# linum-uqam/ViT-OCM-WMSegmentation

Measured on NVIDIA B200. Metric: sliding_window_seg_megapixels_per_s, higher is better.
Workload: dtype fp16

## Files before the change

### vit-ocm-wmsegmentation_b200/csrc/attention_quad_sm100.cuh

```cuda
#pragma once
#include "attention_sm100.cuh"

namespace vitocm {

constexpr int AQ_PIPES = 4;
constexpr int AQ_BKV = 64;
constexpr int AQ_RING = 5;
constexpr int AQ_TILE_BYTES = AQ_BKV * ATT_DH * 2;
constexpr int AQ_Q_BYTES = ATT_BQ * ATT_DH * 2;
constexpr int AQ_THREADS = (4 * AQ_PIPES + 4) * 32;
constexpr int AQ_PIPE_SMEM = AQ_Q_BYTES + AQ_RING * AQ_TILE_BYTES;
constexpr int AQ_PIPE_BARS = 128;
constexpr int AQ_SMEM_BYTES = AQ_PIPES * (AQ_PIPE_SMEM + AQ_PIPE_BARS) + 64 + 1024 ;
constexpr int AQ_REGS_SOFTMAX = 104;
constexpr int AQ_REGS_CTRL = 64;
static_assert(16 * AQ_REGS_SOFTMAX + 4 * AQ_REGS_CTRL <= 20 * 96, "quad attention: setmaxnreg budgets exceed the launch allocation");
static_assert(AQ_SMEM_BYTES <= 227 * 1024, "quad attention: shared memory");
constexpr int AQ_S_COL = 0;
constexpr int AQ_O_COL = 64;

__device__ __forceinline__ void aq_decode(const AttnArgs& a, int it, int& pair0, int& qt, int& nslots) {
  if (a.group_items == 0) {
    pair0 = it / a.n_fullq;
    qt = it - pair0 * a.n_fullq;
    nslots = 1;
    return;
  }
  const int g = it / a.group_items, r = it - g * a.group_items;
  if (r < a.pack * a.n_fullq) {
    const int pi = r / a.n_fullq;
    pair0 = g * a.pack + pi;
    qt = r - pi * a.n_fullq;
    nslots = 1;
  } else {
    pair0 = g * a.pack;
    qt = a.n_fullq;
    nslots = a.pack;
  }
}
template <int NS, int SL>
__device__ __forceinline__ void aq_slot_mask(uint32_t (&m)[4]) {
#pragma unroll
  for (int w = 0; w < 4; ++w) m[w] = ((NS == 4 ? w : (NS == 2 ? (w >> 1) : 0)) == SL) ? 0u : 0xffffffffu;
}

template <bool F16, bool TL = false>
__global__ void __launch_bounds__(AQ_THREADS, 1)
attn_fwd_quad_kernel(const __grid_constant__ CUtensorMap tmap_q , const __grid_constant__ CUtensorMap tmap_kv ,
                     const __grid_constant__ CUtensorMap tmap_q32 , const AttnArgs args) {
  extern __shared__ __align__(1024) uint8_t smem_raw[];
  const uint32_t smem = (ptx::smem_u32(smem_raw) + 1023u) & ~1023u;
  const uint32_t bars0 = smem + AQ_PIPES * AQ_PIPE_SMEM;
  const uint32_t tmem_ptr_smem = bars0 + AQ_PIPES * AQ_PIPE_BARS;
  const int warp = threadIdx.x >> 5;
  const int lane = threadIdx.x & 31;
  const int N = args.n_tokens;
  const int D = args.embed_dim;
  const int n_kv = (N + AQ_BKV - 1) / AQ_BKV;
  const int p = warp < 4 * AQ_PIPES ? (warp >> 2) : (warp - 4 * AQ_PIPES);
  const uint32_t smem_q = smem + p * AQ_PIPE_SMEM;
  const uint32_t smem_ring = smem_q + AQ_Q_BYTES;
  const uint32_t bars = bars0 + p * AQ_PIPE_BARS;
  const uint32_t q_full = bars;
  const uint32_t s_full = bars + 8;
  const uint32_t p_full = bars + 16;
  const uint32_t o_full = bars + 24;
  const uint32_t o_empty = bars + 32;
  const uint32_t kv_full = bars + 40;
  const uint32_t kv_empty = bars + 80;
  static_assert(80 + 8 * AQ_RING <= AQ_PIPE_BARS, "quad attention: barrier block");

  if (warp == 4 * AQ_PIPES && lane == 0) {
    ptx::prefetch_tmap(&tmap_q);
    ptx::prefetch_tmap(&tmap_kv);
    ptx::prefetch_tmap(&tmap_q32);
    for (int pp = 0; pp < AQ_PIPES; ++pp) {
      const uint32_t b = bars0 + pp * AQ_PIPE_BARS;
      ptx::mbar_init(b, 1);
      ptx::mbar_init(b + 8, 1);
      ptx::mbar_init(b + 16, 4);
      ptx::mbar_init(b + 24, 1);
      ptx::mbar_init(b + 32, 4);
      for (int i = 0; i < AQ_RING; ++i) {
        ptx::mbar_init(b + 40 + 8 * i, 1);
        ptx::mbar_init(b + 80 + 8 * i, 1);
      }
    }
    ptx::fence_barrier_init();
  }
  if (warp == 4 * AQ_PIPES + 1) {
    ptx::tmem_alloc(tmem_ptr_smem, 512);
    ptx::tmem_relinquish();
  }
  if (warp == 4 * AQ_PIPES + 2 && lane == 0 && args.stagger_clk > 0) {
    const long long wait_clk = static_cast<long long>(args.stagger_clk) * blockIdx.x / gridDim.x;
    const long long t0 = clock64();
    while (clock64() - t0 < wait_clk) {}
  }
  ptx::tc_fence_before();
  __syncthreads();
  ptx::tc_fence_after();
  const uint32_t tmem_base = ptx::lds_u32(tmem_ptr_smem) + static_cast<uint32_t>(p * 128);

  const int first = static_cast<int>(blockIdx.x) * AQ_PIPES + p;
  const int stride = static_cast<int>(gridDim.x) * AQ_PIPES;

  if (warp >= 4 * AQ_PIPES) {
    asm volatile("setmaxnreg.dec.sync.aligned.u32 %0;" ::"n"(AQ_REGS_CTRL));
    if (ptx::elect_one()) {
      const uint32_t s_tmem = tmem_base + AQ_S_COL, o_tmem = tmem_base + AQ_O_COL;
      const uint64_t q_desc = ptx::make_smem_desc_sw128(smem_q, 1024, 0);
      auto kv_len_mma = [&](int j) {
        int len = N - j * AQ_BKV;
        len = len > AQ_BKV ? AQ_BKV : len;
        return (len + 15) & ~15;
      };
      auto clamp_pair = [&](int pr) { return pr < args.n_pairs ? pr : args.n_pairs - 1; };
      auto load_q = [&](int it) {
        int pair0, qt, ns;
        aq_decode(args, it, pair0, qt, ns);
        ptx::mbar_arrive_expect_tx(q_full, AQ_Q_BYTES);
        if (ns == 1) {
          const int pair = clamp_pair(pair0);
          const int b = pair / args.heads, h = pair - b * args.heads;
          ptx::tma_load_2d(smem_q, &tmap_q, q_full, h * ATT_DH, b * N + qt * ATT_BQ);
        } else {
          const int per = 4 / ns;
          for (int u = 0; u < 4; ++u) {
            const int pr = clamp_pair(pair0 + u / per);
            const int b = pr / args.heads, h = pr - b * args.heads;
            ptx::tma_load_2d(smem_q + u * 4096, &tmap_q32, q_full, h * ATT_DH, b * N + qt * ATT_BQ + (u % per) * 32);
          }
        }
      };
      int loaded = 0, used = 0;
      int l_it = first, l_j = 0, l_which = 1, l_sl = 0, l_ns = 1;
      int l_col = 0, l_row = 0;
      auto set_load_coords = [&]() {
        if (l_it < args.n_items) {
          int pair0, qt;
          aq_decode(args, l_it, pair0, qt, l_ns);
          const int pr = clamp_pair(pair0 + l_sl);
          const int b = pr / args.heads;
          l_col = (pr - b * args.heads) * ATT_DH;
          l_row = b * N;
        }
      };
      set_load_coords();
      auto fill = [&]() {
        while (loaded - used < AQ_RING && l_it < args.n_items) {
          const int slot = loaded % AQ_RING;
          if (loaded >= AQ_RING) ptx::mbar_wait(kv_empty + 8 * slot, ((loaded / AQ_RING) - 1) & 1, 50);
          ptx::mbar_arrive_expect_tx(kv_full + 8 * slot, AQ_TILE_BYTES);
          ptx::tma_load_2d(smem_ring + slot * AQ_TILE_BYTES, &tmap_kv, kv_full + 8 * slot, l_which * D + l_col, l_row + l_j * AQ_BKV);
          ++loaded;
          bool recode = l_ns > 1;
          if (++l_sl == l_ns) {
            l_sl = 0;
            if (l_which == 1) {
              l_which = 2;
            } else {
              l_which = 1;
              if (++l_j == n_kv) { l_j = 0; l_it += stride; recode = true; }
            }
          }
          if (recode) set_load_coords();
        }
      };
      if (first < args.n_items) load_q(first);
      fill();
      auto issue_s = [&](int j, int nslots) {
        const uint32_t idesc = ptx::make_idesc(ATT_BQ, kv_len_mma(j), false, false, F16 ? 0u : 1u);
        if (nslots == 1) {
          const int slot = used % AQ_RING;
          ptx::mbar_wait(kv_full + 8 * slot, (used / AQ_RING) & 1, 52);
          ptx::tc_fence_after();
          const uint64_t k_desc = ptx::make_smem_desc_sw128(smem_ring + slot * AQ_TILE_BYTES, 1024, 0);
#pragma unroll
          for (int k = 0; k < ATT_DH / 16; ++k)
            ptx::umma_bf16_ss(s_tmem, ptx::desc_advance(q_desc, k * 32), ptx::desc_advance(k_desc, k * 32), idesc, k ? 1u : 0u);
          ptx::umma_commit(kv_empty + 8 * slot);
          ++used;
        } else {
          auto slot_s = [&](auto ns_tag, auto sl_tag) {
            if (loaded <= used) fill();
            const int slot = used % AQ_RING;
            ptx::mbar_wait(kv_full + 8 * slot, (used / AQ_RING) & 1, 56);
            ptx::tc_fence_after();
            const uint64_t k_desc = ptx::make_smem_desc_sw128(smem_ring + slot * AQ_TILE_BYTES, 1024, 0);
            uint32_t lm[4];
            aq_slot_mask<decltype(ns_tag)::value, decltype(sl_tag)::value>(lm);
#pragma unroll
            for (int k = 0; k < ATT_DH / 16; ++k)
              ptx::umma_bf16_ss_masked(s_tmem, ptx::desc_advance(q_desc, k * 32), ptx::desc_advance(k_desc, k * 32), idesc, k ? 1u : 0u, lm);
            ptx::umma_commit(kv_empty + 8 * slot);
            ++used;
          };
          using I0 = std::integral_constant<int, 0>; using I1 = std::integral_constant<int, 1>;
          using I2 = std::integral_constant<int, 2>; using I3 = std::integral_constant<int, 3>; using I4 = std::integral_constant<int, 4>;
          if (nslots == 2) { slot_s(I2{}, I0{}); slot_s(I2{}, I1{}); }
          else { slot_s(I4{}, I0{}); slot_s(I4{}, I1{}); slot_s(I4{}, I2{}); slot_s(I4{}, I3{}); }
        }
        ptx::umma_commit(s_full);
      };
      int g = 0;
      int w = 0;
      for (int it = first; it < args.n_items; it += stride, ++w) {
        const bool tl = TL && args.timeline != nullptr && blockIdx.x == 0 && p < 2 && w == args.timeline_item;
        int nslots, pair0_unused, qt_unused;
        aq_decode(args, it, pair0_unused, qt_unused, nslots);
        ptx::mbar_wait(q_full, w & 1, 51);
        issue_s(0, nslots);
        if constexpr (TL) att_stamp(args, tl, 1, 0, 0, p);
        for (int j = 0; j < n_kv; ++j, ++g) {
          fill();
          constexpr uint32_t idesc_pv = ptx::make_idesc(ATT_BQ, ATT_DH, false,  true, F16 ? 0u : 1u);
          const int ksteps = kv_len_mma(j) / 16;
          const uint32_t acc0 = j > 0 ? 1u : 0u;
          if (nslots == 1 && args.ctrl_hoist) {
            const bool more = j + 1 < n_kv;
            const int slot_v = used % AQ_RING, slot_k = (used + 1) % AQ_RING;
            ptx::mbar_wait(kv_full + 8 * slot_v, (used / AQ_RING) & 1, 55);
            if (more) ptx::mbar_wait(kv_full + 8 * slot_k, ((used + 1) / AQ_RING) & 1, 52);
            const uint64_t v_desc = ptx::make_smem_desc_sw128(smem_ring + slot_v * AQ_TILE_BYTES, 1024, 1024);
            const uint64_t k_desc = ptx::make_smem_desc_sw128(smem_ring + slot_k * AQ_TILE_BYTES, 1024, 0);
            const uint32_t idesc_s = ptx::make_idesc(ATT_BQ, kv_len_mma(more ? j + 1 : j), false, false, F16 ? 0u : 1u);
            const uint32_t bar_v = kv_empty + 8 * slot_v, bar_k = kv_empty + 8 * slot_k;
            if (j == 0 && w > 0) ptx::mbar_wait(o_empty, (w - 1) & 1, 54);
            ptx::mbar_wait(p_full, g & 1, 53);
            ptx::tc_fence_after();
            if constexpr (TL) att_stamp(args, tl, 1, j, 1, p);
            if (ksteps == AQ_BKV / 16) {
#pragma unroll
              for (int k = 0; k < AQ_BKV / 16; ++k)
                ptx::umma_bf16_ts(o_tmem, s_tmem + k * 8, ptx::desc_advance(v_desc, k * 2048), idesc_pv, k ? 1u : acc0);
            } else {
#pragma unroll 1
              for (int k = 0; k < ksteps; ++k)
                ptx::umma_bf16_ts(o_tmem, s_tmem + k * 8, ptx::desc_advance(v_desc, k * 2048), idesc_pv, k ? 1u : acc0);
            }
            ptx::umma_commit(bar_v);
            if constexpr (TL) att_stamp(args, tl, 1, j, 2, p);
            if (more) {
#pragma unroll
              for (int k = 0; k < ATT_DH / 16; ++k)
                ptx::umma_bf16_ss(s_tmem, ptx::desc_advance(q_desc, k * 32), ptx::desc_advance(k_desc, k * 32), idesc_s, k ? 1u : 0u);
              ptx::umma_commit(bar_k);
              ptx::umma_commit(s_full);
              used += 2;
              if constexpr (TL) att_stamp(args, tl, 1, j + 1, 0, p);
            } else {
              ptx::umma_commit(o_full);
              ++used;
              if (it + stride < args.n_items) load_q(it + stride);
            }
            continue;
          }
          ptx::mbar_wait(p_full, g & 1, 53);
          ptx::tc_fence_after();
          if constexpr (TL) att_stamp(args, tl, 1, j, 1, p);
          if (j == 0 && w > 0) {
            ptx::mbar_wait(o_empty, (w - 1) & 1, 54);
            ptx::tc_fence_after();
          }
          if (nslots == 1) {
            const int slot = used % AQ_RING;
            ptx::mbar_wait(kv_full + 8 * slot, (used / AQ_RING) & 1, 55);
            ptx::tc_fence_after();
            const uint64_t v_desc = ptx::make_smem_desc_sw128(smem_ring + slot * AQ_TILE_BYTES, 1024, 1024);
#pragma unroll 1
            for (int k = 0; k < ksteps; ++k)
              ptx::umma_bf16_ts(o_tmem, s_tmem + k * 8, ptx::desc_advance(v_desc, k * 2048), idesc_pv, k ? 1u : acc0);
            ptx::umma_commit(kv_empty + 8 * slot);
            ++used;
            if (j == n_kv - 1) ptx::umma_commit(o_full);
          } else {
            auto slot_pv = [&](auto ns_tag, auto sl_tag) {
              if (loaded <= used) fill();
              const int slot = used % AQ_RING;
              ptx::mbar_wait(kv_full + 8 * slot, (used / AQ_RING) & 1, 57);
              ptx::tc_fence_after();
              const uint64_t v_desc = ptx::make_smem_desc_sw128(smem_ring + slot * AQ_TILE_BYTES, 1024, 1024);
              uint32_t lm[4];
              aq_slot_mask<decltype(ns_tag)::value, decltype(sl_tag)::value>(lm);
              if (ksteps == AQ_BKV / 16) {
#pragma unroll
                for (int k = 0; k < AQ_BKV / 16; ++k)
                  ptx::umma_bf16_ts_masked(o_tmem, s_tmem + k * 8, ptx::desc_advance(v_desc, k * 2048), idesc_pv, k ? 1u : acc0, lm);
              } else {
#pragma unroll 1
                for (int k = 0; k < ksteps; ++k)
                  ptx::umma_bf16_ts_masked(o_tmem, s_tmem + k * 8, ptx::desc_advance(v_desc, k * 2048), idesc_pv, k ? 1u : acc0, lm);
              }
              ptx::umma_commit(kv_empty + 8 * slot);
              ++used;
            };
            using I0 = std::integral_constant<int, 0>; using I1 = std::integral_constant<int, 1>;
            using I2 = std::integral_constant<int, 2>; using I3 = std::integral_constant<int, 3>; using I4 = std::integral_constant<int, 4>;
            if (nslots == 2) { slot_pv(I2{}, I0{}); slot_pv(I2{}, I1{}); }
            else { slot_pv(I4{}, I0{}); slot_pv(I4{}, I1{}); slot_pv(I4{}, I2{}); slot_pv(I4{}, I3{}); }
            if (j == n_kv - 1) ptx::umma_commit(o_full);
          }
          if constexpr (TL) att_stamp(args, tl, 1, j, 2, p);
          if (j + 1 < n_kv) {
            issue_s(j + 1, nslots);
            if constexpr (TL) att_stamp(args, tl, 1, j + 1, 0, p);
          } else if (it + stride < args.n_items) {
            load_q(it + stride);
          }
        }
      }
    }
  } else {
    asm volatile("setmaxnreg.inc.sync.aligned.u32 %0;" ::"n"(AQ_REGS_SOFTMAX));
    const int q = warp & 3;
    const int r = q * 32 + lane;
    const uint32_t lane_addr = tmem_base + (static_cast<uint32_t>(q * 32) << 16);
    const float sl2 = args.scale_log2;
    const uint64_t sl2_2 = ptx::dup_f32x2(sl2);
    int g = 0, w = 0;
    for (int it = first; it < args.n_items; it += stride, ++w) {
      const bool tl = TL && args.timeline != nullptr && blockIdx.x == 0 && p < 2 && q == 0 && lane == 0 && w == args.timeline_item;
      float m_used = -INFINITY;
      float l_run = 0.f;
      for (int j = 0; j < n_kv; ++j, ++g) {
        int kv_len = N - j * AQ_BKV;
        kv_len = kv_len > AQ_BKV ? AQ_BKV : kv_len;
        const int nchunks = (((kv_len + 15) & ~15) + 31) >> 5;
        if constexpr (TL) att_stamp(args, tl, 0, j, 0, p);
        ptx::mbar_wait(s_full, g & 1, 60);
        ptx::tc_fence_after();
        if constexpr (TL) att_stamp(args, tl, 0, j, 1, p);
        float bsum = 0.f;
#pragma unroll
        for (int c = 0; c < 2; ++c) {
          if (c < nchunks) {
            uint32_t s[32];
            ptx::tmem_ld_32x32b_x32(lane_addr + AQ_S_COL + c * 32, s);
            ptx::tmem_ld_wait(s);
            if constexpr (TL) att_stamp(args, tl, 0, j, 2 + 2 * c, p);
            if (kv_len < AQ_BKV) {
#pragma unroll
              for (int i = 0; i < 32; ++i)
                if (c * 32 + i >= kv_len) s[i] = 0xff800000u;
            }
            auto chunk_max = [&]() {
              float m0 = fmaxf(__uint_as_float(s[0]), __uint_as_float(s[1]));
#pragma unroll
              for (int i = 2; i < 32; i += 2) m0 = fmaxf(fmaxf(m0, __uint_as_float(s[i])), __uint_as_float(s[i + 1]));
              return m0;
            };
            if (j == 0 && c == 0) m_used = chunk_max();
            float csum;
            auto run_exps = [&]() {
              const uint64_t nm2 = ptx::dup_f32x2(-m_used * sl2);
              uint64_t sum2[2] = {0ull, 0ull};
              uint32_t ph[16];
#pragma unroll
              for (int i = 0; i < 16; ++i) {
                const uint64_t a2 = ptx::fma_f32x2(ptx::pack_f32x2(__uint_as_float(s[2 * i]), __uint_as_float(s[2 * i + 1])), sl2_2, nm2);
                float a0, a1;
                ptx::unpack_f32x2(a2, a0, a1);
                const float e0 = ptx::ex2_approx(a0), e1 = ptx::ex2_approx(a1);
                sum2[i & 1] = ptx::add_f32x2(sum2[i & 1], ptx::pack_f32x2(e0, e1));
                ph[i] = ptx::pack_h2<F16>(e0, e1);
              }
              ptx::tmem_st_32x32b_x16(lane_addr + AQ_S_COL + c * 16, ph);
              float a0, a1, b0, b1;
              ptx::unpack_f32x2(sum2[0], a0, a1);
              ptx::unpack_f32x2(sum2[1], b0, b1);
              csum = (a0 + a1) + (b0 + b1);
            };
            run_exps();
            if ((j > 0 || c > 0) && __any_sync(0xffffffffu, !(csum <= (F16 ? ATT_SUM_TRIGGER_F16 : ATT_SUM_TRIGGER)))) {
              const float m_new = fmaxf(m_used, chunk_max());
              const float a = ptx::ex2_approx((m_used - m_new) * sl2);
              m_used = m_new;
              l_run *= a;
              bsum *= a;
              if (j > 0) {
#pragma unroll 1
                for (int oc = 0; oc < ATT_DH; oc += 8) {
                  uint32_t t[8];
                  ptx::tmem_ld_32x32b_x8(lane_addr + AQ_O_COL + oc, t);
                  ptx::tmem_ld_wait8(t);
#pragma unroll
                  for (int i = 0; i < 8; ++i) t[i] = __float_as_uint(__uint_as_float(t[i]) * a);
                  ptx::tmem_st_32x32b_x8(lane_addr + AQ_O_COL + oc, t);
                }
              }
              if (c > 0) {
                ptx::tmem_st_wait();
#pragma unroll 1
                for (int pc = 0; pc < 16; pc += 8) {
                  uint32_t t[8];
                  ptx::tmem_ld_32x32b_x8(lane_addr + AQ_S_COL + pc, t);
                  ptx::tmem_ld_wait8(t);
#pragma unroll
                  for (int i = 0; i < 8; ++i) {
                    const float lo = ptx::h16_to_f32(F16, static_cast<unsigned short>(t[i] & 0xffffu)) * a;
                    const float hi = ptx::h16_to_f32(F16, static_cast<unsigned short>(t[i] >> 16)) * a;
                    t[i] = ptx::pack_h2<F16>(lo, hi);
                  }
                  ptx::tmem_st_32x32b_x8(lane_addr + AQ_S_COL + pc, t);
                }
              }
              run_exps();
            }
            bsum += csum;
            if constexpr (TL) { if (tl) asm volatile("" ::"f"(csum)); }
            if constexpr (TL) att_stamp(args, tl, 0, j, 3 + 2 * c, p);
          }
        }
        l_run += bsum;
        ptx::tmem_st_wait();
        ptx::tc_fence_before();
        __syncwarp();
        if (lane == 0) ptx::mbar_arrive(p_full);
        if constexpr (TL) att_stamp(args, tl, 0, j, 6, p);
      }
      ptx::mbar_wait(o_full, w & 1, 61);
      ptx::tc_fence_after();
      const float inv = 1.0f / l_run;
      uint32_t t[ATT_DH / 32][32];
#pragma unroll
      for (int c = 0; c < ATT_DH / 32; ++c) ptx::tmem_ld_32x32b_x32(lane_addr + AQ_O_COL + c * 32, t[c]);
#pragma unroll
      for (int c = 0; c < ATT_DH / 32; ++c) ptx::tmem_ld_wait(t[c]);
      ptx::tc_fence_before();
      __syncwarp();
      if (lane == 0) ptx::mbar_arrive(o_empty);
      int pair, qrow;
      {
        int pair0, qt, ns;
        aq_decode(args, it, pair0, qt, ns);
        const int slot_rows = ATT_BQ / ns, sl = r / slot_rows;
        pair = pair0 + sl;
        qrow = qt * ATT_BQ + (r - sl * slot_rows);
      }
      const bool row_ok = pair < args.n_pairs && qrow < N;
      if (!row_ok) pair = 0;
      const int b = pair / args.heads, h = pair - b * args.heads;
      __nv_bfloat16* o = args.out + static_cast<long long>(b * N + qrow) * args.ldo + h * ATT_DH;
      if (row_ok)
#pragma unroll
      for (int c = 0; c < ATT_DH / 32; ++c) {
#pragma unroll
        for (int q4 = 0; q4 < 4; ++q4) {
          float v[8];
#pragma unroll
          for (int i = 0; i < 8; ++i) v[i] = __uint_as_float(t[c][8 * q4 + i]) * inv;
          reinterpret_cast<uint4*>(o + c * 32)[q4] = make_uint4(ptx::pack_h2<F16>(v[0], v[1]), ptx::pack_h2<F16>(v[2], v[3]),
                                                               ptx::pack_h2<F16>(v[4], v[5]), ptx::pack_h2<F16>(v[6], v[7]));
        }
      }
    }
  }

  ptx::tc_fence_before();
  __syncthreads();
  if (warp == 4 * AQ_PIPES + 1) {
    ptx::tc_fence_after();
    ptx::tmem_dealloc(ptx::lds_u32(tmem_ptr_smem), 512);
  }
}

}
```

### vit-ocm-wmsegmentation_b200/csrc/attention_sm100.cuh

```cuda
#pragma once
#include <type_traits>

#include "ptx.cuh"

namespace vitocm {

struct AttnArgs {
  int n_items;
  int n_qtiles, heads;
  int n_fullq;
  int pack;
  int group_items;
  int n_pairs;
  int n_tokens;
  int embed_dim;
  int lo_col_off;
  float scale_log2;
  __nv_bfloat16* out;
  long long ldo;
  int out_lo_off;
  float* lse2;
  int track_max;
  int n_full_items;
  int ctrl_hoist;
  int tails_only;
  int timeline_item;
  long long* timeline;
  int stagger_clk;
};

constexpr int ATT_TL_EVENTS = 8;
constexpr int ATT_TL_BLOCKS = 16;
__device__ __forceinline__ void att_stamp(const AttnArgs& args, bool on, int role, int j, int ev, int pipe = -1) {
  if (pipe < 0) pipe = blockIdx.x;
  if (on && j < ATT_TL_BLOCKS) args.timeline[((pipe * 2 + role) * ATT_TL_BLOCKS + j) * ATT_TL_EVENTS + ev] = clock64();
}

constexpr int ATT_BQ = 128;
constexpr int ATT_BKV = 128;
constexpr int ATT_DH = 64;
constexpr int ATT_THREADS = 256;
constexpr int ATT_TILE_BYTES = 128 * 64 * 2;
#ifndef VITOCM_ATT_RING
#define VITOCM_ATT_RING 3
#endif
constexpr int ATT_RING = VITOCM_ATT_RING;
constexpr int ATT_S_COL = 0;
constexpr int ATT_O_COL = 128;
constexpr int ATT_P_COL = 192;
constexpr float ATT_RESCALE_THRESHOLD = 8.0f;
constexpr float ATT_REDO_THRESHOLD = 60.0f;
constexpr float ATT_REDO_THRESHOLD_F16 = 14.0f;
constexpr float ATT_SUM_TRIGGER = 1.2676506e30f;
constexpr float ATT_SUM_TRIGGER_F16 = 16384.0f;
constexpr int ATT_POLY_DEFAULT = 0;

template <bool SPLIT, int DH = 64>
struct AttnCfg {
  static_assert(DH == 64 || DH == 128, "head_dim 64 or 128");
  static constexpr int ATOMS = DH / 64;
  static constexpr int NPART = SPLIT ? 2 : 1;
  static constexpr int PART_BYTES = ATT_TILE_BYTES * ATOMS;
  static constexpr int SLOT_BYTES = PART_BYTES * NPART;
  static constexpr int Q_BYTES = PART_BYTES * NPART;
  static constexpr int RING = (DH == 128 && SPLIT) ? 2 : ATT_RING;
  static constexpr int SMEM_BYTES = Q_BYTES + RING * SLOT_BYTES + 1024 + 256;
  static constexpr bool ONE_CTA = SPLIT || DH == 128;
  static constexpr int TMEM_COLS = ONE_CTA ? 512 : 256;
  static constexpr int O_COL = ATT_O_COL;
  static constexpr int P_COL = ATT_O_COL + DH;
  static constexpr int REGS_SOFTMAX = ONE_CTA ? 240 : 208;
  static constexpr int REGS_OTHER = ONE_CTA ? 64 : 48;
};

template <bool PACKED>
__device__ __forceinline__ bool att_decode(const AttnArgs& a, int it, int& qt, int& pair0, bool& packed) {
  if (a.tails_only) {
    pair0 = it * a.pack;
    qt = a.n_fullq;
    packed = PACKED && a.pack > 1;
    return pair0 < a.n_pairs;
  }
  if (!PACKED) {
    pair0 = it / a.n_qtiles;
    qt = it - pair0 * a.n_qtiles;
    packed = false;
    return true;
  }
  const int grp = it / a.group_items, r = it - grp * a.group_items;
  if (r < a.pack * a.n_fullq) {
    const int pi = r / a.n_fullq;
    pair0 = grp * a.pack + pi;
    qt = r - pi * a.n_fullq;
    packed = false;
  } else {
    pair0 = grp * a.pack;
    qt = a.n_fullq;
    packed = a.pack > 1;
  }
  return pair0 < a.n_pairs;
}
__device__ __forceinline__ void att_slot_mask(int s, int nslots, uint32_t (&m)[4]) {
#pragma unroll
  for (int w = 0; w < 4; ++w) m[w] = ((nslots == 4 ? w : (w >> 1)) == s) ? 0u : 0xffffffffu;
}

template <bool SPLIT, uint32_t POLY_MASK, bool PACKED, bool F16 = false, int DH = 64>
// ... 482 lines not shown
```

### vit-ocm-wmsegmentation_b200/csrc/vitocm_api.cu

```cuda
#include "../../include/vitocm.h"

#include <cuda.h>
#include <cuda_runtime.h>

#include <atomic>
#include <climits>
#include <cstdarg>
#include <cstdio>
#include <cstdlib>
#include <cstring>
#include <map>
#include <string>
#include <vector>

#include "attention_bwd_sm100.cuh"
#include "attention_sm100.cuh"
#include "gemm_sm100.cuh"
#include "attention_quad_sm100.cuh"
#include "mlp_fused_sm100.cuh"
#include "block_tail_sm100.cuh"
#include "post_kernels.cuh"
#include "train_kernels.cuh"
#include "vit_kernels.cuh"
#include "wgrad_sm100.cuh"
// ... 513 lines not shown
  const float* vecs[8] = {bp, ln2w, ln2b, b1, b2, lnn_w, lnn_b, bqkv};
  for (int i = 0; i < 8; ++i) {
    if (i < 5 && vecs[i] == nullptr) return 1;
    if ((reinterpret_cast<uintptr_t>(vecs[i]) & 15) != 0) return 1;
  }
  if ((lnn_w == nullptr) != (lnn_b == nullptr)) return 1;
  const bool with_qkv = Wqkv != nullptr;
  if (with_qkv && (lnn_w == nullptr || bqkv == nullptr || QKV == nullptr)) return 1;
  if (!with_qkv && lnn_w != nullptr && XN == nullptr) return 1;
  ProfScope prof(PC_TAIL, st);
  CUtensorMap ta, twp, tw1, tw2, tx, txn, twqkv, tqkv;
  const int w2_rows = D == 384 ? 96 : 64;
  TRY(make_tmap_bf16(&ta, CTX, M, D, ld_ctx, GEMM_BM));
  TRY(make_tmap_bf16(&twp, Wp, D, D, ldwp, w2_rows));
  TRY(make_tmap_bf16(&tw1, W1, Hd, D, ldw1, 64));
  TRY(make_tmap_bf16(&tw2, W2, D, Hd, ldw2, w2_rows));
  TRY(make_tmap(&tx, X, true, D, M, D, 32, 32, CU_TENSOR_MAP_SWIZZLE_128B));
  if (lnn_w != nullptr && !with_qkv) TRY(make_tmap(&txn, XN, false, ld_xn, M, ld_xn, 32, 32, CU_TENSOR_MAP_SWIZZLE_64B));
  else txn = tx;
  if (with_qkv) {
    TRY(make_tmap_bf16(&twqkv, Wqkv, 3LL * D, D, ldwqkv, 64));
    TRY(make_tmap_bf16(&tqkv, QKV, M, 3LL * D, ld_qkv, 32));
  } else {
    twqkv = tw1; tqkv = ta;
  }
  TailArgs a{};
  a.M = M; a.hidden = Hd; a.gelu5 = e->f16 ? 1 : 0;
  a.bias_p = bp; a.ln2_w = ln2w; a.ln2_b = ln2b; a.bias1 = b1; a.bias2 = b2; a.lnn_w = lnn_w; a.lnn_b = lnn_b; a.ln_eps = eps;
  a.bias_qkv = bqkv; a.n_qkv_chunks = with_qkv ? 3 * D / MLP_HC : 0;
  a.fold2 = fold2 ? 1 : 0; a.foldn = (foldn && with_qkv) ? 1 : 0;
  a.timeline = timeline;
  { static const int dbg = [] { const char* v = getenv("VITOCM_TAIL_DEBUG"); return v ? atoi(v) : 0; }(); a.debug = dbg; }
  {
    static const int stg = [] { const char* v = getenv("VITOCM_TAIL_STAGGER"); return v ? atoi(v) : -1; }();
    if (stg >= 0) {
      a.stagger_clk = stg;
    } else {
      const long long items = (static_cast<long long>(M) + 2 * GEMM_BM - 1) / (2 * GEMM_BM);
      const long long pairs = e->num_sms / 2;
      const long long r = items % pairs, rounds = (items + pairs - 1) / pairs;
      const double late = (r > 0 ? static_cast<double>(r - 1) : static_cast<double>(pairs - 1)) / static_cast<double>(pairs);
      const double work = static_cast<double>(D) * (D + 2.0 * Hd + (with_qkv ? 3.0 * D : 0.0));
      a.stagger_clk = (items > pairs && late <= 0.04 * static_cast<double>(rounds)) ? static_cast<int>(105000.0 * work / (384.0 * (384.0 + 3072.0 + 1152.0))) : 0;
    }
  }
  { static const int tli = [] { const char* v = getenv("VITOCM_MLP_TL_ITEM"); return v ? atoi(v) : 1; }(); a.timeline_item = tli; }
  if (D == 384) return e->f16 ? launch_block_tail<6, true>(ta, twp, tw1, tw2, tx, txn, twqkv, tqkv, a, e->num_sms, st) : launch_block_tail<6, false>(ta, twp, tw1, tw2, tx, txn, twqkv, tqkv, a, e->num_sms, st);
  return e->f16 ? launch_block_tail<2, true>(ta, twp, tw1, tw2, tx, txn, twqkv, tqkv, a, e->num_sms, st) : launch_block_tail<2, false>(ta, twp, tw1, tw2, tx, txn, twqkv, tqkv, a, e->num_sms, st);
}

int run_attention(const vitocm_engine* e, const void* qkv, long long ld, int B, int N, void* ctx, long long ldo, cudaStream_t st,
                  long long* timeline = nullptr, float* lse2 = nullptr) {
  const int D = e->cfg.embed_dim, H = e->cfg.num_heads;
  const bool hd128 = D == 128 * H;
  const long long M = static_cast<long long>(B) * N;
  ProfScope prof(PC_ATTN, st);
  CUtensorMap tq, tq32;
  TRY(make_tmap_bf16(&tq, qkv, M, 3LL * D * e->parts, ld, 128));
  TRY(make_tmap_bf16(&tq32, qkv, M, 3LL * D * e->parts, ld, 32));
  AttnArgs a{};
  a.n_tokens = N; a.embed_dim = D; a.lo_col_off = 3 * D;
  a.scale_log2 = e->cfg.qk_scale * 1.44269504088896340736f;
  a.out = reinterpret_cast<__nv_bfloat16*>(ctx); a.ldo = ldo; a.out_lo_off = D; a.timeline = timeline; a.lse2 = lse2;
  { static const int tli = [] { const char* v = getenv("VITOCM_ATTN_TL_ITEM"); return v ? atoi(v) : 0; }(); a.timeline_item = tli; }
  { static const int tm = [] { const char* v = getenv("VITOCM_ATTN_TRACK_MAX"); return v ? atoi(v) : 0; }(); a.track_max = tm; }
  a.n_qtiles = (N + ATT_BQ - 1) / ATT_BQ; a.heads = H;
  static const int pack_on = [] { const char* v = getenv("VITOCM_ATTN_PACK"); return v ? atoi(v) : 1; }();
  const int tail = N % ATT_BQ;
  a.n_fullq = N / ATT_BQ;
  a.pack = (!pack_on || tail == 0 || tail > 64 || a.n_fullq > 16) ? 1 : (tail > 32 ? 2 : 4);
  a.group_items = a.pack * a.n_fullq + (tail != 0 ? 1 : 0);
  a.n_pairs = B * H;
  const long long items = static_cast<long long>((a.n_pairs + a.pack - 1) / a.pack) * a.group_items;
  if (items > 0x7fffffffLL) return fail(VITOCM_ERR_INVALID, "attention: too many work items");
  a.n_items = static_cast<int>(items);
  static const int quad = [] { const char* v = getenv("VITOCM_ATTN_QUAD"); return v ? atoi(v) : 1; }();
  if (quad && !hd128 && !e->split && lse2 == nullptr && a.n_fullq >= 1) {
    const long long full_items = static_cast<long long>(a.n_pairs) * a.n_fullq;
    if (full_items > 0x7fffffffLL) return fail(VITOCM_ERR_INVALID, "attention: too many work items");
    AttnArgs aq = a;
    aq.n_full_items = static_cast<int>(full_items);
    static const int quad_tails = [] { const char* v = getenv("VITOCM_ATTN_QUAD_TAILS"); return v ? atoi(v) : 1; }();
    const bool tails_here = quad_tails && a.pack > 1;
    static const int quad_pack = [] { const char* v = getenv("VITOCM_ATTN_QUAD_PACK"); return v ? atoi(v) : 2; }();
    aq.group_items = 0;
    { static const int hoist = [] { const char* v = getenv("VITOCM_ATTN_HOIST"); return v ? atoi(v) : 1; }(); aq.ctrl_hoist = hoist; }
    { static const int stg = [] { const char* v = getenv("VITOCM_ATTN_STAGGER"); return v ? atoi(v) : 0; }(); aq.stagger_clk = stg; }
    aq.n_items = aq.n_full_items;
    if (tails_here) {
      aq.pack = (quad_pack == 4 && a.pack == 4) ? 4 : 2;
      aq.group_items = aq.pack * a.n_fullq + 1;
      const long long gi = static_cast<long long>((a.n_pairs + aq.pack - 1) / aq.pack) * aq.group_items;
      if (gi > 0x7fffffffLL) return fail(VITOCM_ERR_INVALID, "attention: too many work items");
      aq.n_items = static_cast<int>(gi);
    }
    CUtensorMap tkv;
    TRY(make_tmap_bf16(&tkv, qkv, M, 3LL * D * e->parts, ld, AQ_BKV));
    const int ctas = (aq.n_items + AQ_PIPES - 1) / AQ_PIPES;
    const dim3 qgrid(ctas < e->num_sms ? ctas : e->num_sms);
    auto qlaunch = [&](auto kern, bool& attr) -> int {
      if (!attr) { CUDA_TRY(cudaFuncSetAttribute(kern, cudaFuncAttributeMaxDynamicSharedMemorySize, AQ_SMEM_BYTES)); attr = true; }
      kern<<<qgrid, AQ_THREADS, AQ_SMEM_BYTES, st>>>(tq, tkv, tq32, aq);
      return 0;
    };
    static bool qattr[4] = {false, false, false, false};
    int qrc;
    if (timeline != nullptr) qrc = e->f16 ? qlaunch(attn_fwd_quad_kernel<true, true>, qattr[3]) : qlaunch(attn_fwd_quad_kernel<false, true>, qattr[2]);
    else qrc = e->f16 ? qlaunch(attn_fwd_quad_kernel<true, false>, qattr[1]) : qlaunch(attn_fwd_quad_kernel<false, false>, qattr[0]);
    if (qrc) return qrc;
    LAUNCH_CHECK();
    if (tail == 0 || tails_here) return 0;
    a.tails_only = 1;
    a.timeline = nullptr;
    a.n_items = (a.n_pairs + a.pack - 1) / a.pack;
  }
  const int resident = e->num_sms * ((e->split || hd128) ? 1 : 2);
  static const int persist = [] { const char* v = getenv("VITOCM_ATTN_PERSISTENT"); return v ? atoi(v) : 1; }();
  const dim3 grid(persist && a.n_items > resident ? resident : a.n_items);
  auto launch = [&](auto kern, int smem_bytes, bool& attr) -> int {
    if (!attr) { CUDA_TRY(cudaFuncSetAttribute(kern, cudaFuncAttributeMaxDynamicSharedMemorySize, smem_bytes)); attr = true; }
    kern<<<grid, ATT_THREADS, smem_bytes, st>>>(tq, tq32, a);
    return 0;
  };
  if (hd128) {
    static bool attr128[8] = {false, false, false, false, false, false, false, false};
    if (a.pack > 1) {
      if (e->split) {
        if (e->f16) TRY(launch(attn_fwd_tcgen05_kernel<true, 0u, true, true, 128>, AttnCfg<true, 128>::SMEM_BYTES, attr128[1]));
        else TRY(launch(attn_fwd_tcgen05_kernel<true, 0u, true, false, 128>, AttnCfg<true, 128>::SMEM_BYTES, attr128[3]));
      } else if (e->f16) TRY(launch(attn_fwd_tcgen05_kernel<false, 0u, true, true, 128>, AttnCfg<false, 128>::SMEM_BYTES, attr128[2]));
      else TRY(launch(attn_fwd_tcgen05_kernel<false, 0u, true, false, 128>, AttnCfg<false, 128>::SMEM_BYTES, attr128[0]));
    } else {
      if (e->split) {
        if (e->f16) TRY(launch(attn_fwd_tcgen05_kernel<true, 0u, false, true, 128>, AttnCfg<true, 128>::SMEM_BYTES, attr128[5]));
        else TRY(launch(attn_fwd_tcgen05_kernel<true, 0u, false, false, 128>, AttnCfg<true, 128>::SMEM_BYTES, attr128[7]));
      } else if (e->f16) TRY(launch(attn_fwd_tcgen05_kernel<false, 0u, false, true, 128>, AttnCfg<false, 128>::SMEM_BYTES, attr128[6]));
      else TRY(launch(attn_fwd_tcgen05_kernel<false, 0u, false, false, 128>, AttnCfg<false, 128>::SMEM_BYTES, attr128[4]));
    }
    LAUNCH_CHECK();
    return 0;
  }
  static bool attr[8] = {false, false, false, false, false, false, false, false};
  if (a.pack > 1) {
    if (e->split) {
      if (e->f16) TRY(launch(attn_fwd_tcgen05_kernel<true, 0u, true, true>, AttnCfg<true>::SMEM_BYTES, attr[1]));
      else TRY(launch(attn_fwd_tcgen05_kernel<true, 0u, true, false>, AttnCfg<true>::SMEM_BYTES, attr[3]));
    } else if (e->f16) TRY(launch(attn_fwd_tcgen05_kernel<false, 0u, true, true>, AttnCfg<false>::SMEM_BYTES, attr[2]));
    else TRY(launch(attn_fwd_tcgen05_kernel<false, 0u, true, false>, AttnCfg<false>::SMEM_BYTES, attr[0]));
  } else {
    if (e->split) {
      if (e->f16) TRY(launch(attn_fwd_tcgen05_kernel<true, 0u, false, true>, AttnCfg<true>::SMEM_BYTES, attr[5]));
      else TRY(launch(attn_fwd_tcgen05_kernel<true, 0u, false, false>, AttnCfg<true>::SMEM_BYTES, attr[7]));
    } else if (e->f16) TRY(launch(attn_fwd_tcgen05_kernel<false, 0u, false, true>, AttnCfg<false>::SMEM_BYTES, attr[6]));
    else TRY(launch(attn_fwd_tcgen05_kernel<false, 0u, false, false>, AttnCfg<false>::SMEM_BYTES, attr[4]));
  }
  LAUNCH_CHECK();
  return 0;
}

int run_layernorm(const float* X, const float* g, const float* b, void* out_bf16, long long ldo, int split, int lo_off,
                  float* out_f32, long long ldf, int M, int D, float eps, cudaStream_t st, float* x_copy = nullptr, int f16 = 0) {
  if (M <= 0) return 0;
  if (D % 4 != 0 || D > LN_MAX_VEC * 128) return fail(VITOCM_ERR_INVALID, "LayerNorm D=%d unsupported", D);
  ProfScope prof(PC_LN, st);
  const int rows_per_block = 8;
  const dim3 grid((M + rows_per_block - 1) / rows_per_block), block(rows_per_block * 32);
  __nv_bfloat16* ob = reinterpret_cast<__nv_bfloat16*>(out_bf16);
  if (D == 384) layernorm_kernel<3><<<grid, block, 0, st>>>(X, g, b, ob, ldo, split, lo_off, out_f32, ldf, M, D, eps, x_copy, f16);
  else if (D == 768) layernorm_kernel<6><<<grid, block, 0, st>>>(X, g, b, ob, ldo, split, lo_off, out_f32, ldf, M, D, eps, x_copy, f16);
  else if (D == 128) layernorm_kernel<1><<<grid, block, 0, st>>>(X, g, b, ob, ldo, split, lo_off, out_f32, ldf, M, D, eps, x_copy, f16);
  else layernorm_kernel<0><<<grid, block, 0, st>>>(X, g, b, ob, ldo, split, lo_off, out_f32, ldf, M, D, eps, x_copy, f16);
  LAUNCH_CHECK();
  return 0;
// ... 1009 lines not shown
```

Before: 229.4.

## Split S MMA into two 32-column halves to overlap softmax with next QK

Measured after the change: 230.6, median of 6. About the same (+0.5%).

```diff
diff --git a/vit-ocm-wmsegmentation_b200/csrc/attention_quad_sm100.cuh b/vit-ocm-wmsegmentation_b200/csrc/attention_quad_sm100.cuh
--- a/vit-ocm-wmsegmentation_b200/csrc/attention_quad_sm100.cuh
+++ b/vit-ocm-wmsegmentation_b200/csrc/attention_quad_sm100.cuh
@@ -10,7 +10,7 @@
 constexpr int AQ_Q_BYTES = ATT_BQ * ATT_DH * 2;
 constexpr int AQ_THREADS = (4 * AQ_PIPES + 4) * 32;
 constexpr int AQ_PIPE_SMEM = AQ_Q_BYTES + AQ_RING * AQ_TILE_BYTES;
-constexpr int AQ_PIPE_BARS = 128;
+constexpr int AQ_PIPE_BARS = 136;
 constexpr int AQ_SMEM_BYTES = AQ_PIPES * (AQ_PIPE_SMEM + AQ_PIPE_BARS) + 64 + 1024 ;
 constexpr int AQ_REGS_SOFTMAX = 104;
 constexpr int AQ_REGS_CTRL = 64;
@@ -41,7 +41,7 @@
 template <int NS, int SL>
 __device__ __forceinline__ void aq_slot_mask(uint32_t (&m)[4]) {
 #pragma unroll
-  for (int w = 0; w < 4; ++w) m[w] = ((NS == 4 ? w : (NS == 2 ? (w >> 1) : 0)) == SL) ? 0u : 0xffffffffu;
+  for (int w = 0; w < 4; ++w) m[w] = ((NS == 2 ? (w >> 1) : 0) == SL) ? 0u : 0xffffffffu;
 }
 
 template <bool F16, bool TL = false>
@@ -62,13 +62,15 @@
   const uint32_t smem_ring = smem_q + AQ_Q_BYTES;
   const uint32_t bars = bars0 + p * AQ_PIPE_BARS;
   const uint32_t q_full = bars;
-  const uint32_t s_full = bars + 8;
-  const uint32_t p_full = bars + 16;
-  const uint32_t o_full = bars + 24;
-  const uint32_t o_empty = bars + 32;
-  const uint32_t kv_full = bars + 40;
-  const uint32_t kv_empty = bars + 80;
-  static_assert(80 + 8 * AQ_RING <= AQ_PIPE_BARS, "quad attention: barrier block");
+  const uint32_t s_full0 = bars + 8;
+  const uint32_t s_full1 = bars + 16;
+  const uint32_t p_full = bars + 24;
+  const uint32_t o_full = bars + 32;
+  const uint32_t o_empty = bars + 40;
+  const uint32_t s_half_free = bars + 48;
+  const uint32_t kv_full = bars + 56;
+  const uint32_t kv_empty = bars + 96;
+  static_assert(96 + 8 * AQ_RING <= AQ_PIPE_BARS, "quad attention: barrier block");
 
   if (warp == 4 * AQ_PIPES && lane == 0) {
     ptx::prefetch_tmap(&tmap_q);
@@ -78,12 +80,14 @@
       const uint32_t b = bars0 + pp * AQ_PIPE_BARS;
       ptx::mbar_init(b, 1);
       ptx::mbar_init(b + 8, 1);
-      ptx::mbar_init(b + 16, 4);
-      ptx::mbar_init(b + 24, 1);
-      ptx::mbar_init(b + 32, 4);
+      ptx::mbar_init(b + 16, 1);
+      ptx::mbar_init(b + 24, 4);
+      ptx::mbar_init(b + 32, 1);
+      ptx::mbar_init(b + 40, 4);
+      ptx::mbar_init(b + 48, 4);
       for (int i = 0; i < AQ_RING; ++i) {
-        ptx::mbar_init(b + 40 + 8 * i, 1);
-        ptx::mbar_init(b + 80 + 8 * i, 1);
+        ptx::mbar_init(b + 56 + 8 * i, 1);
+        ptx::mbar_init(b + 96 + 8 * i, 1);
       }
     }
     ptx::fence_barrier_init();
@@ -169,146 +173,112 @@
       };
       if (first < args.n_items) load_q(first);
       fill();
-      auto issue_s = [&](int j, int nslots) {
-        const uint32_t idesc = ptx::make_idesc(ATT_BQ, kv_len_mma(j), false, false, F16 ? 0u : 1u);
-        if (nslots == 1) {
-          const int slot = used % AQ_RING;
-          ptx::mbar_wait(kv_full + 8 * slot, (used / AQ_RING) & 1, 52);
+      constexpr uint32_t idesc_pv = ptx::make_idesc(ATT_BQ, ATT_DH, false,  true, F16 ? 0u : 1u);
+      auto idesc_s = [](int n) { return ptx::make_idesc(ATT_BQ, n, false, false, F16 ? 0u : 1u); };
+      auto ring_desc = [&](int pos, uint32_t lbo) {
+        const int slot = pos % AQ_RING;
+        ptx::mbar_wait(kv_full + 8 * slot, (pos / AQ_RING) & 1, 52);
+        return ptx::make_smem_desc_sw128(smem_ring + slot * AQ_TILE_BYTES, 1024, lbo);
+      };
+      auto release = [&](int pos) { ptx::umma_commit(kv_empty + 8 * (pos % AQ_RING)); };
+      using I0 = std::integral_constant<int, 0>; using I1 = std::integral_constant<int, 1>; using I2 = std::integral_constant<int, 2>;
+      auto run_item = [&](auto ns_tag, int it, int g, int w, bool tl) {
+        constexpr int NS = decltype(ns_tag)::value;
+        auto slots = [&](auto f) { f(I0{}); if constexpr (NS == 2) f(I1{}); };
+        auto mma_s = [&](auto sl_tag, uint32_t col, uint64_t k_desc, uint32_t idesc) {
+          if constexpr (NS == 1) {
+#pragma unroll
+            for (int k = 0; k < ATT_DH / 16; ++k)
+              ptx::umma_bf16_ss(s_tmem + col, ptx::desc_advance(q_desc, k * 32), ptx::desc_advance(k_desc, k * 32), idesc, k ? 1u : 0u);
+          } else {
+            uint32_t lm[4];
+            aq_slot_mask<NS, decltype(sl_tag)::value>(lm);
+#pragma unroll
+            for (int k = 0; k < ATT_DH / 16; ++k)
+              ptx::umma_bf16_ss_masked(s_tmem + col, ptx::desc_advance(q_desc, k * 32), ptx::desc_advance(k_desc, k * 32), idesc, k ? 1u : 0u, lm);
+          }
+        };
+        auto mma_pv = [&](auto sl_tag, uint32_t col, uint64_t v_desc, int ksteps, uint32_t acc0) {
+          [[maybe_unused]] uint32_t lm[4];
+          if constexpr (NS == 2) aq_slot_mask<NS, decltype(sl_tag)::value>(lm);
+          auto step = [&](int k) {
+            if constexpr (NS == 1)
+              ptx::umma_bf16_ts(o_tmem, s_tmem + col + k * 8, ptx::desc_advance(v_desc, k * 2048), idesc_pv, k ? 1u : acc0);
+            else
+              ptx::umma_bf16_ts_masked(o_tmem, s_tmem + col + k * 8, ptx::desc_advance(v_desc, k * 2048), idesc_pv, k ? 1u : acc0, lm);
+          };
+          if (ksteps == AQ_BKV / 16) {
+#pragma unroll
+            for (int k = 0; k < AQ_BKV / 16; ++k) step(k);
+          } else {
+#pragma unroll 1
+            for (int k = 0; k < ksteps; ++k) step(k);
+          }
+        };
+        {
+          const int len = kv_len_mma(0);
+          uint64_t kd[NS];
+          ptx::mbar_wait(q_full, w & 1, 51);
+          slots([&](auto sl) { kd[decltype(sl)::value] = ring_desc(used + decltype(sl)::value, 0); });
           ptx::tc_fence_after();
-          const uint64_t k_desc = ptx::make_smem_desc_sw128(smem_ring + slot * AQ_TILE_BYTES, 1024, 0);
-#pragma unroll
-          for (int k = 0; k < ATT_DH / 16; ++k)
-            ptx::umma_bf16_ss(s_tmem, ptx::desc_advance(q_desc, k * 32), ptx::desc_advance(k_desc, k * 32), idesc, k ? 1u : 0u);
-          ptx::umma_commit(kv_empty + 8 * slot);
-          ++used;
-        } else {
-          auto slot_s = [&](auto ns_tag, auto sl_tag) {
-            if (loaded <= used) fill();
-            const int slot = used % AQ_RING;
-            ptx::mbar_wait(kv_full + 8 * slot, (used / AQ_RING) & 1, 56);
+          slots([&](auto sl) { mma_s(sl, 0, kd[decltype(sl)::value], idesc_s(len < 32 ? len : 32)); });
+          ptx::umma_commit(s_full0);
+          if (len > 32) slots([&](auto sl) { mma_s(sl, 32, ptx::desc_advance(kd[decltype(sl)::value], 4096), idesc_s(len - 32)); });
+          ptx::umma_commit(s_full1);
+          slots([&](auto sl) { release(used + decltype(sl)::value); });
+          used += NS;
+          if constexpr (TL) att_stamp(args, tl, 1, 0, 0, p);
+        }
+        for (int j = 0; j < n_kv; ++j) {
+          fill();
+          const int gj = g + j;
+          const bool more = j + 1 < n_kv;
+          const uint32_t h = (j & 1) * 32;
+          const int ln = more ? kv_len_mma(j + 1) : 0;
+          uint64_t vd[NS], kd[NS];
+          slots([&](auto sl) {
+            constexpr int SL = decltype(sl)::value;
+            vd[SL] = ring_desc(used + SL, 1024);
+            if (more) kd[SL] = ring_desc(used + NS + SL, 0);
+          });
+          const uint32_t idesc0 = idesc_s(ln < 32 ? ln : 32), idesc1 = idesc_s(ln > 32 ? ln - 32 : 32);
+          const int ksteps = kv_len_mma(j) / 16;
+          if (j == 0 && w > 0) ptx::mbar_wait(o_empty, (w - 1) & 1, 54);
+          if (more) {
+            ptx::mbar_wait(s_half_free, (gj - w) & 1, 58);
             ptx::tc_fence_after();
-            const uint64_t k_desc = ptx::make_smem_desc_sw128(smem_ring + slot * AQ_TILE_BYTES, 1024, 0);
-            uint32_t lm[4];
-            aq_slot_mask<decltype(ns_tag)::value, decltype(sl_tag)::value>(lm);
-#pragma unroll
-            for (int k = 0; k < ATT_DH / 16; ++k)
-              ptx::umma_bf16_ss_masked(s_tmem, ptx::desc_advance(q_desc, k * 32), ptx::desc_advance(k_desc, k * 32), idesc, k ? 1u : 0u, lm);
-            ptx::umma_commit(kv_empty + 8 * slot);
-            ++used;
-          };
-          using I0 = std::integral_constant<int, 0>; using I1 = std::integral_constant<int, 1>;
-          using I2 = std::integral_constant<int, 2>; using I3 = std::integral_constant<int, 3>; using I4 = std::integral_constant<int, 4>;
-          if (nslots == 2) { slot_s(I2{}, I0{}); slot_s(I2{}, I1{}); }
-          else { slot_s(I4{}, I0{}); slot_s(I4{}, I1{}); slot_s(I4{}, I2{}); slot_s(I4{}, I3{}); }
-        }
-        ptx::umma_commit(s_full);
+            if constexpr (TL) att_stamp(args, tl, 1, j, 3, p);
+            slots([&](auto sl) { mma_s(sl, 32 - h, kd[decltype(sl)::value], idesc0); });
+            ptx::umma_commit(s_full0);
+            if constexpr (TL) att_stamp(args, tl, 1, j + 1, 4, p);
+          }
+          ptx::mbar_wait(p_full, gj & 1, 53);
+          ptx::tc_fence_after();
+          if constexpr (TL) att_stamp(args, tl, 1, j, 1, p);
+          slots([&](auto sl) { mma_pv(sl, h, vd[decltype(sl)::value], ksteps, j > 0 ? 1u : 0u); });
+          slots([&](auto sl) { release(used + decltype(sl)::value); });
+          if constexpr (TL) att_stamp(args, tl, 1, j, 2, p);
+          if (more) {
+            if (ln > 32) slots([&](auto sl) { mma_s(sl, h, ptx::desc_advance(kd[decltype(sl)::value], 4096), idesc1); });
+            ptx::umma_commit(s_full1);
+            slots([&](auto sl) { release(used + NS + decltype(sl)::value); });
+            used += 2 * NS;
+            if constexpr (TL) att_stamp(args, tl, 1, j + 1, 0, p);
+          } else {
+            ptx::umma_commit(o_full);
+            used += NS;
+            if (it + stride < args.n_items) load_q(it + stride);
+          }
+        }
       };
       int g = 0;
       int w = 0;
-      for (int it = first; it < args.n_items; it += stride, ++w) {
+      for (int it = first; it < args.n_items; it += stride, ++w, g += n_kv) {
         const bool tl = TL && args.timeline != nullptr && blockIdx.x == 0 && p < 2 && w == args.timeline_item;
         int nslots, pair0_unused, qt_unused;
         aq_decode(args, it, pair0_unused, qt_unused, nslots);
-        ptx::mbar_wait(q_full, w & 1, 51);
-        issue_s(0, nslots);
-        if constexpr (TL) att_stamp(args, tl, 1, 0, 0, p);
-        for (int j = 0; j < n_kv; ++j, ++g) {
-          fill();
-          constexpr uint32_t idesc_pv = ptx::make_idesc(ATT_BQ, ATT_DH, false,  true, F16 ? 0u : 1u);
-          const int ksteps = kv_len_mma(j) / 16;
-          const uint32_t acc0 = j > 0 ? 1u : 0u;
-          if (nslots == 1 && args.ctrl_hoist) {
-            const bool more = j + 1 < n_kv;
-            const int slot_v = used % AQ_RING, slot_k = (used + 1) % AQ_RING;
-            ptx::mbar_wait(kv_full + 8 * slot_v, (used / AQ_RING) & 1, 55);
-            if (more) ptx::mbar_wait(kv_full + 8 * slot_k, ((used + 1) / AQ_RING) & 1, 52);
-            const uint64_t v_desc = ptx::make_smem_desc_sw128(smem_ring + slot_v * AQ_TILE_BYTES, 1024, 1024);
-            const uint64_t k_desc = ptx::make_smem_desc_sw128(smem_ring + slot_k * AQ_TILE_BYTES, 1024, 0);
-            const uint32_t idesc_s = ptx::make_idesc(ATT_BQ, kv_len_mma(more ? j + 1 : j), false, false, F16 ? 0u : 1u);
-            const uint32_t bar_v = kv_empty + 8 * slot_v, bar_k = kv_empty + 8 * slot_k;
-            if (j == 0 && w > 0) ptx::mbar_wait(o_empty, (w - 1) & 1, 54);
-            ptx::mbar_wait(p_full, g & 1, 53);
-            ptx::tc_fence_after();
-            if constexpr (TL) att_stamp(args, tl, 1, j, 1, p);
-            if (ksteps == AQ_BKV / 16) {
-#pragma unroll
-              for (int k = 0; k < AQ_BKV / 16; ++k)
-                ptx::umma_bf16_ts(o_tmem, s_tmem + k * 8, ptx::desc_advance(v_desc, k * 2048), idesc_pv, k ? 1u : acc0);
-            } else {
-#pragma unroll 1
-              for (int k = 0; k < ksteps; ++k)
-                ptx::umma_bf16_ts(o_tmem, s_tmem + k * 8, ptx::desc_advance(v_desc, k * 2048), idesc_pv, k ? 1u : acc0);
-            }
-            ptx::umma_commit(bar_v);
-            if constexpr (TL) att_stamp(args, tl, 1, j, 2, p);
-            if (more) {
-#pragma unroll
-              for (int k = 0; k < ATT_DH / 16; ++k)
-                ptx::umma_bf16_ss(s_tmem, ptx::desc_advance(q_desc, k * 32), ptx::desc_advance(k_desc, k * 32), idesc_s, k ? 1u : 0u);
-              ptx::umma_commit(bar_k);
-              ptx::umma_commit(s_full);
-              used += 2;
-              if constexpr (TL) att_stamp(args, tl, 1, j + 1, 0, p);
-            } else {
-              ptx::umma_commit(o_full);
-              ++used;
-              if (it + stride < args.n_items) load_q(it + stride);
-            }
-            continue;
-          }
-          ptx::mbar_wait(p_full, g & 1, 53);
-          ptx::tc_fence_after();
-          if constexpr (TL) att_stamp(args, tl, 1, j, 1, p);
-          if (j == 0 && w > 0) {
-            ptx::mbar_wait(o_empty, (w - 1) & 1, 54);
-            ptx::tc_fence_after();
-          }
-          if (nslots == 1) {
-            const int slot = used % AQ_RING;
-            ptx::mbar_wait(kv_full + 8 * slot, (used / AQ_RING) & 1, 55);
-            ptx::tc_fence_after();
-            const uint64_t v_desc = ptx::make_smem_desc_sw128(smem_ring + slot * AQ_TILE_BYTES, 1024, 1024);
-#pragma unroll 1
-            for (int k = 0; k < ksteps; ++k)
-              ptx::umma_bf16_ts(o_tmem, s_tmem + k * 8, ptx::desc_advance(v_desc, k * 2048), idesc_pv, k ? 1u : acc0);
-            ptx::umma_commit(kv_empty + 8 * slot);
-            ++used;
-            if (j == n_kv - 1) ptx::umma_commit(o_full);
-          } else {
-            auto slot_pv = [&](auto ns_tag, auto sl_tag) {
-              if (loaded <= used) fill();
-              const int slot = used % AQ_RING;
-              ptx::mbar_wait(kv_full + 8 * slot, (used / AQ_RING) & 1, 57);
-              ptx::tc_fence_after();
-              const uint64_t v_desc = ptx::make_smem_desc_sw128(smem_ring + slot * AQ_TILE_BYTES, 1024, 1024);
-              uint32_t lm[4];
-              aq_slot_mask<decltype(ns_tag)::value, decltype(sl_tag)::value>(lm);
-              if (ksteps == AQ_BKV / 16) {
-#pragma unroll
-                for (int k = 0; k < AQ_BKV / 16; ++k)
-                  ptx::umma_bf16_ts_masked(o_tmem, s_tmem + k * 8, ptx::desc_advance(v_desc, k * 2048), idesc_pv, k ? 1u : acc0, lm);
-              } else {
-#pragma unroll 1
-                for (int k = 0; k < ksteps; ++k)
-                  ptx::umma_bf16_ts_masked(o_tmem, s_tmem + k * 8, ptx::desc_advance(v_desc, k * 2048), idesc_pv, k ? 1u : acc0, lm);
-              }
-              ptx::umma_commit(kv_empty + 8 * slot);
-              ++used;
-            };
-            using I0 = std::integral_constant<int, 0>; using I1 = std::integral_constant<int, 1>;
-            using I2 = std::integral_constant<int, 2>; using I3 = std::integral_constant<int, 3>; using I4 = std::integral_constant<int, 4>;
-            if (nslots == 2) { slot_pv(I2{}, I0{}); slot_pv(I2{}, I1{}); }
-            else { slot_pv(I4{}, I0{}); slot_pv(I4{}, I1{}); slot_pv(I4{}, I2{}); slot_pv(I4{}, I3{}); }
-            if (j == n_kv - 1) ptx::umma_commit(o_full);
-          }
-          if constexpr (TL) att_stamp(args, tl, 1, j, 2, p);
-          if (j + 1 < n_kv) {
-            issue_s(j + 1, nslots);
-            if constexpr (TL) att_stamp(args, tl, 1, j + 1, 0, p);
-          } else if (it + stride < args.n_items) {
-            load_q(it + stride);
-          }
-        }
+        if (nslots == 1) run_item(I1{}, it, g, w, tl);
+        else run_item(I2{}, it, g, w, tl);
       }
     }
   } else {
@@ -327,17 +297,28 @@
         int kv_len = N - j * AQ_BKV;
         kv_len = kv_len > AQ_BKV ? AQ_BKV : kv_len;
         const int nchunks = (((kv_len + 15) & ~15) + 31) >> 5;
+        const uint32_t h = (j & 1) * 32;
         if constexpr (TL) att_stamp(args, tl, 0, j, 0, p);
-        ptx::mbar_wait(s_full, g & 1, 60);
+        ptx::mbar_wait(s_full0, g & 1, 60);
         ptx::tc_fence_after();
         if constexpr (TL) att_stamp(args, tl, 0, j, 1, p);
         float bsum = 0.f;
 #pragma unroll
         for (int c = 0; c < 2; ++c) {
           if (c < nchunks) {
+            if (c == 1) {
+              ptx::mbar_wait(s_full1, g & 1, 62);
+              ptx::tc_fence_after();
+              if constexpr (TL) att_stamp(args, tl, 0, j, 7, p);
+            }
             uint32_t s[32];
-            ptx::tmem_ld_32x32b_x32(lane_addr + AQ_S_COL + c * 32, s);
+            ptx::tmem_ld_32x32b_x32(lane_addr + AQ_S_COL + (c ? 32 - h : h), s);
             ptx::tmem_ld_wait(s);
+            if (c == 1 && j + 1 < n_kv) {
+              ptx::tc_fence_before();
+              __syncwarp();
+              if (lane == 0) ptx::mbar_arrive(s_half_free);
+            }
             if constexpr (TL) att_stamp(args, tl, 0, j, 2 + 2 * c, p);
             if (kv_len < AQ_BKV) {
 #pragma unroll
@@ -365,7 +346,7 @@
                 sum2[i & 1] = ptx::add_f32x2(sum2[i & 1], ptx::pack_f32x2(e0, e1));
                 ph[i] = ptx::pack_h2<F16>(e0, e1);
               }
-              ptx::tmem_st_32x32b_x16(lane_addr + AQ_S_COL + c * 16, ph);
+              ptx::tmem_st_32x32b_x16(lane_addr + AQ_S_COL + h + c * 16, ph);
               float a0, a1, b0, b1;
               ptx::unpack_f32x2(sum2[0], a0, a1);
               ptx::unpack_f32x2(sum2[1], b0, b1);
@@ -379,6 +360,10 @@
               l_run *= a;
               bsum *= a;
               if (j > 0) {
+                if (c == 0) {
+                  ptx::mbar_wait(s_full1, g & 1, 63);
+                  ptx::tc_fence_after();
+                }
 #pragma unroll 1
                 for (int oc = 0; oc < ATT_DH; oc += 8) {
                   uint32_t t[8];
@@ -394,7 +379,7 @@
 #pragma unroll 1
                 for (int pc = 0; pc < 16; pc += 8) {
                   uint32_t t[8];
-                  ptx::tmem_ld_32x32b_x8(lane_addr + AQ_S_COL + pc, t);
+                  ptx::tmem_ld_32x32b_x8(lane_addr + AQ_S_COL + h + pc, t);
                   ptx::tmem_ld_wait8(t);
 #pragma unroll
                   for (int i = 0; i < 8; ++i) {
@@ -402,7 +387,7 @@
                     const float hi = ptx::h16_to_f32(F16, static_cast<unsigned short>(t[i] >> 16)) * a;
                     t[i] = ptx::pack_h2<F16>(lo, hi);
                   }
-                  ptx::tmem_st_32x32b_x8(lane_addr + AQ_S_COL + pc, t);
+                  ptx::tmem_st_32x32b_x8(lane_addr + AQ_S_COL + h + pc, t);
                 }
               }
               run_exps();
@@ -412,6 +397,7 @@
             if constexpr (TL) att_stamp(args, tl, 0, j, 3 + 2 * c, p);
           }
         }
+        if (nchunks == 1) ptx::mbar_wait(s_full1, g & 1, 62);
         l_run += bsum;
         ptx::tmem_st_wait();
         ptx::tc_fence_before();
diff --git a/vit-ocm-wmsegmentation_b200/csrc/attention_sm100.cuh b/vit-ocm-wmsegmentation_b200/csrc/attention_sm100.cuh
--- a/vit-ocm-wmsegmentation_b200/csrc/attention_sm100.cuh
+++ b/vit-ocm-wmsegmentation_b200/csrc/attention_sm100.cuh
@@ -22,7 +22,6 @@
   float* lse2;
   int track_max;
   int n_full_items;
-  int ctrl_hoist;
   int tails_only;
   int timeline_item;
   long long* timeline;
diff --git a/vit-ocm-wmsegmentation_b200/csrc/vitocm_api.cu b/vit-ocm-wmsegmentation_b200/csrc/vitocm_api.cu
--- a/vit-ocm-wmsegmentation_b200/csrc/vitocm_api.cu
+++ b/vit-ocm-wmsegmentation_b200/csrc/vitocm_api.cu
@@ -619,13 +619,11 @@
     aq.n_full_items = static_cast<int>(full_items);
     static const int quad_tails = [] { const char* v = getenv("VITOCM_ATTN_QUAD_TAILS"); return v ? atoi(v) : 1; }();
     const bool tails_here = quad_tails && a.pack > 1;
-    static const int quad_pack = [] { const char* v = getenv("VITOCM_ATTN_QUAD_PACK"); return v ? atoi(v) : 2; }();
     aq.group_items = 0;
-    { static const int hoist = [] { const char* v = getenv("VITOCM_ATTN_HOIST"); return v ? atoi(v) : 1; }(); aq.ctrl_hoist = hoist; }
     { static const int stg = [] { const char* v = getenv("VITOCM_ATTN_STAGGER"); return v ? atoi(v) : 0; }(); aq.stagger_clk = stg; }
     aq.n_items = aq.n_full_items;
     if (tails_here) {
-      aq.pack = (quad_pack == 4 && a.pack == 4) ? 4 : 2;
+      aq.pack = 2;
       aq.group_items = aq.pack * a.n_fullq + 1;
       const long long gi = static_cast<long long>((a.n_pairs + aq.pack - 1) / aq.pack) * aq.group_items;
       if (gi > 0x7fffffffLL) return fail(VITOCM_ERR_INVALID, "attention: too many work items");
```
